# Enigmatisms/Distributed-Machine-Learning-Experiment-Document

Measured on AMD Instinct MI355X. Metric: samples/sec (whole node) for task3 DDP CNN at 1/2/4/8 MI355X, higher is better.
Workload: dtype bf16; 1 GPU; model=resnet18, global_batch=1024, per_gpu_batch=1024, image_size=224, parallelism=dp1, optimizer=SGD(momentum=0.9), fused flat, ddp=none (dp1: no communication), backend=native, fused_step=False, hip_graph=False, stream_priority=high, sampler=MySampler(partition)

## Files before the change

### csrc/stem_fused.hip

```cpp
#include <type_traits>

#include "common.h"
#include "igemm_common.h"
#include "kernels.h"

namespace dm {

namespace {

constexpr int SCO = 64;
constexpr int SKP = 176;
constexpr int SKH = 192;
constexpr int RING = 13;

typedef short s4v __attribute__((ext_vector_type(4)));
typedef unsigned int nt4 __attribute__((ext_vector_type(4)));
typedef unsigned int nt2 __attribute__((ext_vector_type(2)));
__device__ __forceinline__ s4v tr4(const unsigned char* p) {
  return __builtin_amdgcn_ds_read_tr16_b64_v4i16((__attribute__((address_space(3))) s4v*)p);
}

struct StemGeo {
  int Hin, Win, Hout, Wout, PH, PW;
  int ROWB;
  int SP;
};

struct RawUnit {
  uint4 w;
};

__device__ __forceinline__ void lds_barrier() {
  asm volatile("s_waitcnt lgkmcnt(0)\n\ts_barrier" ::: "memory");
}

__device__ __forceinline__ int ring_of(int iy) { return (iy + 13 * 8) % RING; }

template <int NT, int RU>
struct RawMap {
  int r[RU], k[RU];
  unsigned valid;
  float sc[RU][4], bi[RU][4];
  __device__ __forceinline__ void init(int t, int Win, const float (&nsc)[3], const float (&nbi)[3]) {
    const int upr = 3 * Win / 4;
#pragma unroll
    for (int u = 0; u < RU; ++u) {
      const int e = t + NT * u;
      r[u] = e < 4 * upr ? e / upr : -1;
      k[u] = e - (e / upr) * upr;
#pragma unroll
      for (int j = 0; j < 4; ++j) {
        const int c = (k[u] + j) % 3;
        sc[u][j] = c == 0 ? nsc[0] : c == 1 ? nsc[1] : nsc[2];
        bi[u][j] = c == 0 ? nbi[0] : c == 1 ? nbi[1] : nbi[2];
      }
    }
  }
  template <int DT>
  __device__ __forceinline__ void load(RawUnit (&ru)[RU], const void* img, long long rowbase, int Hin,
                                       int Win, int iy0, int nrows) {
    valid = 0;
#pragma unroll
    for (int u = 0; u < RU; ++u) {
      const int iy = iy0 + r[u];
      const bool ok = r[u] >= 0 && r[u] < nrows && iy >= 0 && iy < Hin;
      valid |= ok ? 1u << u : 0u;
      const int iyc = min(max(iy, 0), Hin - 1);
      const long long off = rowbase + (long long)iyc * Win * 3 + 4LL * (r[u] >= 0 ? k[u] : 0);
      if (DT == 0) {
        ru[u].w = *reinterpret_cast<const uint4*>(reinterpret_cast<const float*>(img) + off);
      } else if (DT == 1) {
        const uint2 w = *reinterpret_cast<const uint2*>(reinterpret_cast<const bf16_t*>(img) + off);
        ru[u].w = make_uint4(w.x, w.y, 0, 0);
      } else {
        ru[u].w = make_uint4(*reinterpret_cast<const uint32_t*>(reinterpret_cast<const uint8_t*>(img) + off), 0, 0, 0);
      }
    }
  }
  template <int DT>
  __device__ __forceinline__ void store(const RawUnit (&ru)[RU], bf16_t* S, int SP, int nrows) const {
#pragma unroll
    for (int u = 0; u < RU; ++u) {
      if (r[u] < 0 || r[u] >= nrows) continue;
      float x[4];
      const uint4 w = ru[u].w;
      if (DT == 0) {
        x[0] = __uint_as_float(w.x); x[1] = __uint_as_float(w.y);
        x[2] = __uint_as_float(w.z); x[3] = __uint_as_float(w.w);
      } else if (DT == 1) {
        x[0] = __uint_as_float(w.x << 16); x[1] = __uint_as_float(w.x & 0xffff0000u);
        x[2] = __uint_as_float(w.y << 16); x[3] = __uint_as_float(w.y & 0xffff0000u);
      } else {
        x[0] = (float)(w.x & 0xff); x[1] = (float)((w.x >> 8) & 0xff);
        x[2] = (float)((w.x >> 16) & 0xff); x[3] = (float)(w.x >> 24);
      }
      const bool ok = (valid >> u) & 1;
#pragma unroll
      for (int j = 0; j < 4; ++j) x[j] = ok ? fmaf(x[j], sc[u][j], bi[u][j]) : 0.f;
      bf16_t* p = S + r[u] * SP + 4 * k[u] + 9;
      p[0] = f2bf(x[0]);
      *reinterpret_cast<uint32_t*>(p + 1) = pack_bf2(x[1], x[2]);
      p[3] = f2bf(x[3]);
    }
  }
};

struct EMap {
  bool act;
  int soff, eoff;
  int part;
  __device__ __forceinline__ void init(int t, int Wout) {
    act = t < 3 * Wout;
    const int ox = t / 3;
    part = t - 3 * ox;
    soff = 6 * ox + 8 * part;
    eoff = 48 * ox + 16 * part;
  }
  __device__ __forceinline__ void build(unsigned char* E, const bf16_t* S, const StemGeo& G, int iy0,
                                        int nrows, int srow0) const {
    if (!act) return;
    if (nrows == 4) build_n<4>(E, S, G, iy0, srow0);
    else if (nrows == 2) build_n<2>(E, S, G, iy0, srow0);
    else for (int q = 0; q < nrows; ++q) build_n<1>(E, S, G, iy0 + q, srow0 + q);
  }
  template <int NR>
  __device__ __forceinline__ void build_n(unsigned char* E, const bf16_t* S, const StemGeo& G,
                                          int iy0, int srow0) const {
    uint32_t w[NR][4];
#pragma unroll
    for (int q = 0; q < NR; ++q) {
      const int sr = min(max(srow0 + q, 0), 3);
      const uint32_t* sp = reinterpret_cast<const uint32_t*>(S + sr * G.SP + soff);
#pragma unroll
      for (int j = 0; j < 4; ++j) w[q][j] = sp[j];
    }
#pragma unroll
    for (int q = 0; q < NR; ++q) {
      const int iy = iy0 + q;
      const bool in = iy >= 0 && iy < G.Hin;
      uint4 v = make_uint4(in ? w[q][0] : 0u, in ? w[q][1] : 0u, in ? w[q][2] : 0u, in ? w[q][3] : 0u);
      if (part == 2) {
        v.z = in ? (v.z & 0xffffu) | 0x3f800000u : 0u;
        v.w = 0;
      }
      *reinterpret_cast<uint4*>(E + ring_of(iy) * G.ROWB + eoff) = v;
    }
  }
};

__host__ __device__ constexpr unsigned wcode(int kh, int kw) { return (unsigned)((2 - kh) << 2 | (2 - kw)); }

__device__ __forceinline__ uint32_t mono2(uint32_t w) {
  const uint32_t s = (w >> 15) & 0x00010001u;
  return w ^ (s * 0x7fffu);
}

__device__ __forceinline__ int yoff(int slot, int px, int c8, int Wout) {
  return ((slot * Wout + px) * 8 + (c8 ^ ((((px >> 1) & 1) << 2) | ((px >> 2) & 3)))) * 16;
}

template <int PF>
__device__ __forceinline__ f32x16 conv_tile(const bf16x8 (&wa)[11], const unsigned char* E,
                                            const int (&rowoff)[7], int pxoff, bool hh) {
  f32x16 acc;
#pragma unroll
  for (int r = 0; r < 16; ++r) acc[r] = 0.f;
  bf16x8 bq[11];
#pragma unroll
  for (int s = 0; s < 11 + PF; ++s) {
    if (s < 11) {
      const int j0 = 2 * s, j1 = 2 * s + 1;
      const int k0 = j0 / 3 > 6 ? 6 : j0 / 3, k1 = j1 / 3 > 6 ? 6 : j1 / 3;
      const int a0 = rowoff[k0] + 16 * (j0 % 3), a1 = rowoff[k1] + 16 * (j1 % 3);
      bq[s] = *reinterpret_cast<const bf16x8*>(E + (hh ? a1 : a0) + pxoff);
    }
    if (s >= PF) acc = __builtin_amdgcn_mfma_f32_32x32x16_bf16(wa[s - PF], bq[s - PF], acc, 0, 0, 0);
  }
  return acc;
}

__device__ __forceinline__ void ring_rows(int (&ro)[7], int iy0, int ROWB) {
  const int r0 = ring_of(iy0);
#pragma unroll
  for (int r = 0; r < 7; ++r) {
    const int x = r0 + r;
    ro[r] = (x >= RING ? x - RING : x) * ROWB;
  }
}

__device__ __forceinline__ void pair_wgrad(f32x16 (&acc)[3], const unsigned char* T,
                                           const unsigned char* E, const StemGeo& G, int i,
                                           int wid, int lane) {
  const int cb = wid & 1, kq = (wid >> 1) & 1;
  const int g = lane >> 4, h = g >> 1, i16 = lane & 15, q = i16 >> 2, p = i16 & 3;
  const int c8 = 4 * cb + 2 * (g & 1) + (p >> 1);
  int ta[2], ta8[2], boff[2][3];
#pragma unroll
  for (int sl = 0; sl < 2; ++sl) {
    ta[sl] = yoff(sl, 4 * h + q, c8, G.Wout) + 8 * (p & 1);
    ta8[sl] = yoff(sl, 4 * h + q + 8, c8, G.Wout) + 8 * (p & 1);
    const int oy = 2 * i + sl;
#pragma unroll
    for (int u = 0; u < 3; ++u) {
      const int k = 32 * (3 * kq + u) + 16 * (g & 1) + 4 * p;
      int ky = k / 24, kk = k - 24 * ky;
      if (ky > 6) ky = 6;
      boff[sl][u] = ring_of(2 * oy - 3 + ky) * G.ROWB + (4 * h + q) * 48 + 2 * kk;
    }
  }
  struct Stage {
    s4v a0, a1, b0[3], b1[3];
  };
  auto load = [&](Stage& S, int t, int sl) {
    const int mo = 16 * t;
    S.a0 = tr4(T + ta[sl] + mo * 128);
    S.a1 = tr4(T + ta8[sl] + mo * 128);
#pragma unroll
    for (int u = 0; u < 3; ++u) {
      S.b0[u] = tr4(E + boff[sl][u] + mo * 48);
      S.b1[u] = tr4(E + boff[sl][u] + (mo + 8) * 48);
    }
  };
  auto mma = [&](const Stage& S) {
    const bf16x8 af = (bf16x8){S.a0[0], S.a0[1], S.a0[2], S.a0[3], S.a1[0], S.a1[1], S.a1[2], S.a1[3]};
#pragma unroll
    for (int u = 0; u < 3; ++u) {
      const bf16x8 bf = (bf16x8){S.b0[u][0], S.b0[u][1], S.b0[u][2], S.b0[u][3],
                                 S.b1[u][0], S.b1[u][1], S.b1[u][2], S.b1[u][3]};
      acc[u] = __builtin_amdgcn_mfma_f32_32x32x16_bf16(af, bf, acc[u], 0, 0, 0);
    }
  };
  const int nt = G.Wout >> 4;
  Stage s0, s1;
  load(s0, 0, 0);
  for (int t = 0; t < nt; ++t) {
    load(s1, t, 1);
    mma(s0);
    if (t + 1 < nt) load(s0, t + 1, 0);
    mma(s1);
  }
}

}

struct StemFwdArgs {
  const void* img;
  const long long* idx;
  float nsc[3], nbi[3];
  const bf16_t* wk;
  const float* gamma;
  bf16_t* pext;
  uint8_t* code;
  float* stats;
  int N, nimg;
  StemGeo G;
};

constexpr int FNT = 768;
constexpr int FVT = FNT - 256;
constexpr int FRU = 2;

template <int DT>
__global__ void __launch_bounds__(FNT, 1) stem_fwd_kernel(StemFwdArgs a) {
  extern __shared__ __attribute__((aligned(16))) unsigned char smem[];
  const StemGeo G = a.G;
  const int YB = 2 * G.Wout * 128;
  const int SB = 4 * G.SP;
  unsigned char* E = smem;
  unsigned char* Y = E + RING * G.ROWB;
  bf16_t* S = reinterpret_cast<bf16_t*>(Y + 2 * YB);
  const int tid = threadIdx.x, lane = tid & 63, wid = tid >> 6;
  const bool train = a.stats != nullptr;
  {
    const int tot16 = (RING * G.ROWB + 2 * YB + 2 * SB * 2) / 16;
    for (int e = tid; e < tot16; e += FNT) reinterpret_cast<uint4*>(smem)[e] = make_uint4(0, 0, 0, 0);
  }
  __syncthreads();
  const int nimg = a.N > (int)blockIdx.x ? (a.N - 1 - (int)blockIdx.x) / (int)gridDim.x + 1 : 0;
  const int SPI = G.PH + 2;
  const int nsteps = nimg * SPI;
  auto img_base = [&](int q) -> long long {
    const int n = (int)blockIdx.x + q * (int)gridDim.x;
    long long row = a.idx ? a.idx[n] : (long long)n;
    row = row < 0 ? 0 : row >= a.nimg ? a.nimg - 1 : row;
    return row * G.Hin * G.Win * 3;
  };
  const bool mw = wid < 4;
  if (mw) {
    const int slot = wid >> 1, cb = wid & 1, hh = lane >> 5;
    bf16x8 wa[11];
#pragma unroll
    for (int s = 0; s < 11; ++s)
      wa[s] = *reinterpret_cast<const bf16x8*>(a.wk + (32 * cb + (lane & 31)) * SKP + 16 * s + 8 * hh);
    uint32_t flm[4][2];
#pragma unroll
    for (int g4 = 0; g4 < 4; ++g4)
#pragma unroll
      for (int h = 0; h < 2; ++h) {
        const int co = 32 * cb + 8 * g4 + 4 * hh + 2 * h;
        flm[g4][h] = (a.gamma[co] < 0.f ? 0xffffu : 0u) | (a.gamma[co + 1] < 0.f ? 0xffff0000u : 0u);
      }
    float st_s[16], st_q[16];
#pragma unroll
    for (int r = 0; r < 16; ++r) st_s[r] = st_q[r] = 0.f;
    for (int st = 0; st <= nsteps; ++st) {
      lds_barrier();
      if (st == nsteps) break;
      const int kk = st % SPI;
      if (kk < 2) continue;
      const int i = kk - 2;
      unsigned char* Yt = Y + (st & 1) * YB;
      int ro[7];
      ring_rows(ro, 4 * i - 3 + 2 * slot, G.ROWB);
#pragma unroll
      for (int mb = 0; mb < 4; ++mb) {
        if (32 * mb >= G.Wout) break;
        const int px = 32 * mb + (lane & 31);
        const int pxb = min(px, G.Wout - 1);
        f32x16 acc = conv_tile<4>(wa, E, ro, pxb * 48, hh);
        const bool valid = px < G.Wout;
        if (32 * mb + 32 > G.Wout) {
#pragma unroll
          for (int r = 0; r < 16; ++r) acc[r] = valid ? acc[r] : 0.f;
        }
#pragma unroll
        for (int r = 0; r < 16; ++r) {
          st_s[r] += acc[r];
          st_q[r] = fmaf(acc[r], acc[r], st_q[r]);
        }
        if (valid) {
#pragma unroll
          for (int g4 = 0; g4 < 4; ++g4) {
            const uint32_t k0 = mono2(pack_bf2(acc[4 * g4 + 0], acc[4 * g4 + 1])) ^ flm[g4][0];
            const uint32_t k1 = mono2(pack_bf2(acc[4 * g4 + 2], acc[4 * g4 + 3])) ^ flm[g4][1];
            *reinterpret_cast<uint2*>(Yt + yoff(slot, px, 4 * cb + g4, G.Wout) + 8 * hh) = make_uint2(k0, k1);
          }
        }
      }
    }
    if (!train) return;
    float* red = reinterpret_cast<float*>(smem);
    __syncthreads();
#pragma unroll
    for (int r = 0; r < 16; ++r) {
      red[((wid * 2 + 0) * 16 + r) * 64 + lane] = st_s[r];
      red[((wid * 2 + 1) * 16 + r) * 64 + lane] = st_q[r];
    }
    __syncthreads();
    if (tid < 2 * SCO) {
      const int co = tid & 63, which = tid >> 6;
      const int c = co >> 5, cl = co & 31, h = (cl >> 2) & 1, r = (cl & 3) + 4 * (cl >> 3);
      float sum = 0.f;
      for (int sl = 0; sl < 2; ++sl) {
        const float* rp = red + (((2 * sl + c) * 2 + which) * 16 + r) * 64 + 32 * h;
        for (int l = 0; l < 32; ++l) sum += rp[l];
      }
      a.stats[(long long)blockIdx.x * 2 * SCO + which * SCO + co] = sum;
    }
    return;
  }
  const int vt = tid - 256;
  RawMap<FVT, FRU> rm;
  rm.init(vt, G.Win, a.nsc, a.nbi);
  EMap em;
  em.init(vt, G.Wout);
  RawUnit ru[FRU];
  const bool pact = vt < G.PW * 8;
  const int pj = vt >> 3, pc8 = vt & 7;
  uint32_t pflip[4];
#pragma unroll
  for (int k = 0; k < 4; ++k) {
    const int c = pc8 * 8 + 2 * k;
    pflip[k] = (pact && a.gamma[c] < 0.f ? 0xffffu : 0u) |
               (pact && a.gamma[c + 1] < 0.f ? 0xffff0000u : 0u);
  }
  int pv[8];
  long long bcur = nimg > 0 ? img_base(0) : 0, bnext = nimg > 1 ? img_base(1) : 0;
  int bq = 0;
  auto base = [&](int qq) {
    if (qq != bq) {
      bcur = bnext;
      bq = qq;
      bnext = qq + 1 < nimg ? img_base(qq + 1) : 0;
    }
    return bcur;
  };
  auto plan = [&](int t, int& pq, int& piy) -> int {
    if (t >= nsteps) return 0;
    pq = t / SPI;
    const int k = t - pq * SPI;
    if (k == 0) { piy = 0; return 4; }
    if (k == 1) { piy = 4; return 2; }
    if (k - 2 + 1 < G.PH) { piy = 4 * (k - 2) + 6; return 4; }
    return 0;
  };
  int pend = 0;
  if (nimg > 0) {
    rm.load<DT>(ru, a.img, bcur, G.Hin, G.Win, 0, 4);
    rm.store<DT>(ru, S + 1 * SB, G.SP, 4);
    int pq = 0, piy = 0;
    pend = plan(1, pq, piy);
    if (pend) rm.load<DT>(ru, a.img, base(pq), G.Hin, G.Win, piy, pend);
  }
  for (int st = 0; st <= nsteps; ++st) {
    lds_barrier();
    const int q = st / SPI, kk = st - q * SPI;
    if (pend) rm.store<DT>(ru, S + (st & 1) * SB, G.SP, pend);
    {
      int pq = 0, piy = 0;
      pend = plan(st + 2, pq, piy);
      if (pend) rm.load<DT>(ru, a.img, base(pq), G.Hin, G.Win, piy, pend);
    }
    if (st >= 1) {
      const int ps = st - 1, pq = ps / SPI, pk = ps - pq * SPI;
      if (pk >= 2 && pact) {
        const int i = pk - 2;
        const unsigned char* Yt = Y + (ps & 1) * YB;
        if (i == 0) {
#pragma unroll
          for (int c = 0; c < 8; ++c) pv[c] = INT_MIN;
        }
        int hk[2][8];
#pragma unroll
        for (int sl = 0; sl < 2; ++sl) {
          uint4 w[3];
#pragma unroll
          for (int kw = 0; kw < 3; ++kw) {
            const int px = 2 * pj - 1 + kw;
            w[kw] = (px >= 0 && px < G.Wout) ? *reinterpret_cast<const uint4*>(Yt + yoff(sl, px, pc8, G.Wout))
                                             : make_uint4(0x80008000u, 0x80008000u, 0x80008000u, 0x80008000u);
          }
#pragma unroll
          for (int c = 0; c < 8; ++c) {
            const int sh = 16 * (c & 1);
            int k3[3];
#pragma unroll
            for (int kw = 0; kw < 3; ++kw) {
              const uint32_t ww[4] = {w[kw].x, w[kw].y, w[kw].z, w[kw].w};
              const uint32_t d = ww[c >> 1];
              k3[kw] = (int)((sh ? (d & 0xffff0000u) : (d << 16)) | (uint32_t)(2 - kw));
            }
            hk[sl][c] = max(max(k3[0], k3[1]), k3[2]);
          }
        }
        uint32_t o[4] = {0, 0, 0, 0}, cd = 0;
#pragma unroll
        for (int c = 0; c < 8; ++c) {
          const int v = max(max(pv[c] | 8, hk[0][c] | 4), hk[1][c]);
          cd |= ((uint32_t)v & 15u) << (4 * c);
          o[c >> 1] |= ((uint32_t)v >> 16) << (16 * (c & 1));
          pv[c] = hk[1][c];
        }
#pragma unroll
        for (int k = 0; k < 4; ++k) o[k] = mono2(o[k] ^ pflip[k]);
        const int n = (int)blockIdx.x + pq * (int)gridDim.x;
        const long long po = (((long long)n * G.PH + i) * G.PW + pj) * SCO + pc8 * 8;
        __builtin_nontemporal_store((nt4){o[0], o[1], o[2], o[3]}, reinterpret_cast<nt4*>(a.pext + po));
        __builtin_nontemporal_store(cd, reinterpret_cast<uint32_t*>(a.code + po / 2));
      }
    }
    if (st < nsteps) {
      const bf16_t* Sp = S + ((st - 1) & 1) * SB;
      if (kk == 0) em.build(E, Sp, G, -3, 7, -3);
      else if (kk == 1) em.build(E, Sp, G, 4, 2, 0);
      else if (kk - 2 + 1 < G.PH) em.build(E, Sp, G, 4 * (kk - 2) + 6, 4, 0);
    }
  }
  if (train) {
    __syncthreads();
    __syncthreads();
  }
}

__global__ void __launch_bounds__(256) stem_pool_apply_kernel(const bf16_t* __restrict__ pext,
                                                              const uint32_t* __restrict__ code,
                                                              const float* __restrict__ scale,
                                                              const float* __restrict__ shift,
                                                              bf16_t* __restrict__ out,
                                                              uint32_t* __restrict__ code4,
                                                              long long n8) {
  constexpr int U = 4;
  const long long b = (long long)blockIdx.x * 256 * U + threadIdx.x;
  nt4 v[U];
  uint32_t cd[U];
#pragma unroll
  for (int u = 0; u < U; ++u) {
    const long long e = b + 256LL * u;
    if (e < n8) {
      v[u] = __builtin_nontemporal_load(reinterpret_cast<const nt4*>(pext) + e);
      cd[u] = code4 ? __builtin_nontemporal_load(code + e) : 0u;
    }
  }
#pragma unroll
  for (int u = 0; u < U; ++u) {
    const long long e = b + 256LL * u;
    if (e >= n8) continue;
    const int c0 = (int)(e & 7) * 8;
    const uint32_t w[4] = {v[u][0], v[u][1], v[u][2], v[u][3]};
    uint32_t o[4], keep = 0;
#pragma unroll
    for (int k = 0; k < 4; ++k) {
      float r[2];
#pragma unroll
      for (int hlf = 0; hlf < 2; ++hlf) {
        const int c = c0 + 2 * k + hlf;
        const float z = bf2f((bf16_t)((w[k] >> (16 * hlf)) & 0xffff)) * scale[c] + shift[c];
        r[hlf] = z > 0.f ? z : 0.f;
        keep |= z > 0.f ? 15u << (4 * (2 * k + hlf)) : 0u;
      }
      o[k] = pack_bf2(r[0], r[1]);
    }
    __builtin_nontemporal_store((nt4){o[0], o[1], o[2], o[3]}, reinterpret_cast<nt4*>(out) + e);
    if (code4) code4[e] = (cd[u] & keep) | ~keep;
  }
}

constexpr int GK = 192;
constexpr int GONE = 93;
struct WavePlan {
  int nb, blk[4];
  int tcb;
  int nt, kind[5], x[5], y[5];
};
__device__ constexpr WavePlan kPlans[8] = {
    {2, {0, 1, 0, 0}, 0, 5, {0, 0, 0, 1, 1}, {0, 0, 1, 0, 0}, {0, 1, 1, 0, 1}},
    {2, {2, 3, 0, 0}, 0, 5, {0, 0, 0, 1, 1}, {0, 0, 1, 0, 0}, {0, 1, 1, 0, 1}},
    {2, {4, 5, 0, 0}, 0, 5, {0, 0, 0, 1, 1}, {0, 0, 1, 0, 0}, {0, 1, 1, 0, 1}},
    {4, {0, 1, 2, 3}, -1, 4, {0, 0, 0, 0, 0}, {0, 0, 1, 1, 0}, {2, 3, 2, 3, 0}},
    {4, {0, 1, 4, 5}, -1, 4, {0, 0, 0, 0, 0}, {0, 0, 1, 1, 0}, {2, 3, 2, 3, 0}},
    {4, {2, 3, 4, 5}, -1, 4, {0, 0, 0, 0, 0}, {0, 0, 1, 1, 0}, {2, 3, 2, 3, 0}},
    {3, {0, 1, 2, 0}, 1, 3, {1, 1, 1, 0, 0}, {0, 0, 0, 0, 0}, {0, 1, 2, 0, 0}},
    {3, {3, 4, 5, 0}, 1, 3, {1, 1, 1, 0, 0}, {0, 0, 0, 0, 0}, {0, 1, 2, 0, 0}},
};

struct BwdFrags {
  bf16x8 xf[4], tf;
};

template <int W>
__device__ __forceinline__ void gram_slot(f32x16 (&acc)[5], const unsigned char* T,
                                          const unsigned char* E, const StemGeo& G, int i,
                                          int slot, int t0, int t1, int lane) {
  constexpr WavePlan P = kPlans[W];
  const int g = lane >> 4, h = g >> 1, i16 = lane & 15, q = i16 >> 2, p = i16 & 3;
  const int oy = 2 * i + slot;
  int boff[4];
#pragma unroll
  for (int b = 0; b < P.nb; ++b) {
    const int k = 32 * P.blk[b] + 16 * (g & 1) + 4 * p;
    int ky = k / 24;
    const int kk = k - 24 * ky;
    if (ky > 6) ky = 6;
    boff[b] = ring_of(2 * oy - 3 + ky) * G.ROWB + (4 * h + q) * 48 + 2 * kk;
  }
  int ta = 0, ta8 = 0;
  if (P.tcb >= 0) {
    const int c8 = 4 * P.tcb + 2 * (g & 1) + (p >> 1);
    ta = yoff(slot, 4 * h + q, c8, G.Wout) + 8 * (p & 1);
    ta8 = yoff(slot, 4 * h + q + 8, c8, G.Wout) + 8 * (p & 1);
  }
  auto load = [&](BwdFrags& F, int t) {
    const int mo = 16 * t;
#pragma unroll
    for (int b = 0; b < P.nb; ++b) {
      const s4v v0 = tr4(E + boff[b] + mo * 48), v1 = tr4(E + boff[b] + (mo + 8) * 48);
      F.xf[b] = (bf16x8){v0[0], v0[1], v0[2], v0[3], v1[0], v1[1], v1[2], v1[3]};
    }
    if (P.tcb >= 0) {
      const s4v v0 = tr4(T + ta + mo * 128), v1 = tr4(T + ta8 + mo * 128);
      F.tf = (bf16x8){v0[0], v0[1], v0[2], v0[3], v1[0], v1[1], v1[2], v1[3]};
    }
  };
  auto mma = [&](const BwdFrags& F) {
#pragma unroll
    for (int j = 0; j < P.nt; ++j)
      acc[j] = __builtin_amdgcn_mfma_f32_32x32x16_bf16(P.kind[j] ? F.tf : F.xf[P.x[j]], F.xf[P.y[j]],
                                                       acc[j], 0, 0, 0);
  };
  for (int t = t0; t < t1; ++t) {
    BwdFrags f;
    load(f, t);
    mma(f);
  }
}

template <int W>
__device__ __forceinline__ void gram_store(const f32x16 (&acc)[5], float* dslab, float* gslab,
                                           int lane) {
  constexpr WavePlan P = kPlans[W];
#pragma unroll
  for (int j = 0; j < P.nt; ++j)
#pragma unroll
    for (int r = 0; r < 16; ++r) {
      const int row = (r & 3) + 8 * (r >> 2) + 4 * (lane >> 5);
      const int col = 32 * P.blk[P.y[j]] + (lane & 31);
      if (P.kind[j])
        dslab[(long long)blockIdx.x * SCO * SKH + (32 * P.tcb + row) * SKH + col] = acc[j][r];
      else
        gslab[(long long)blockIdx.x * GK * GK + (32 * P.blk[P.x[j]] + row) * GK + col] = acc[j][r];
    }
}

template <int W>
__device__ __forceinline__ void gram_zero(f32x16 (&acc)[5]) {
#pragma unroll
  for (int j = 0; j < 5; ++j)
#pragma unroll
    for (int r = 0; r < 16; ++r) acc[j][r] = 0.f;
}

struct StemBwdArgs2 {
  const void* img;
  const long long* idx;
  float nsc[3], nbi[3];
  const bf16_t* wk;
  const bf16_t* pdy;
  const uint8_t* code4;
  float* dslab;
  float* gslab;
  int N, nimg;
  int split;
  StemGeo G;
};

constexpr int PRING = 3;
constexpr int BNT = 1024;
constexpr int BMW = 8;
constexpr int BVT = BNT - 64 * BMW;

template <int DT>
__global__ void __launch_bounds__(BNT, 1) stem_bwd_kernel(StemBwdArgs2 a) {
  extern __shared__ __attribute__((aligned(16))) unsigned char smem[];
  const StemGeo G = a.G;
  const int TB = 2 * G.Wout * 128;
  unsigned char* E = smem;
  unsigned char* T = E + RING * G.ROWB;
  bf16_t* S = reinterpret_cast<bf16_t*>(T + 2 * TB);
  const int PRB = G.PW * SCO;
  bf16_t* Pg = S + 4 * G.SP;
  uint8_t* Pc = reinterpret_cast<uint8_t*>(Pg + PRING * PRB);
  const int tid = threadIdx.x, lane = tid & 63, wid = tid >> 6;
  {
    const int tot16 = (RING * G.ROWB + 2 * TB + 4 * G.SP * 2) / 16;
    for (int e = tid; e < tot16; e += BNT) reinterpret_cast<uint4*>(smem)[e] = make_uint4(0, 0, 0, 0);
  }
  const int nimg = a.N > (int)blockIdx.x ? (a.N - 1 - (int)blockIdx.x) / (int)gridDim.x + 1 : 0;
  const int SPI = G.PH + 2;
  const int nsteps = nimg * SPI;
  auto img_of = [&](int q) { return (int)blockIdx.x + q * (int)gridDim.x; };
  auto img_base = [&](int q) -> long long {
    long long row = a.idx ? a.idx[img_of(q)] : (long long)img_of(q);
    row = row < 0 ? 0 : row >= a.nimg ? a.nimg - 1 : row;
    return row * G.Hin * G.Win * 3;
  };
  if (wid < BMW) {
    f32x16 acc[5];
    gram_zero<0>(acc);
    __syncthreads();
    EMap em;
    em.init(tid, G.Wout);
    auto run = [&](auto wtag) {
      constexpr int W = decltype(wtag)::value;
      for (int st = 0; st <= nsteps; ++st) {
        lds_barrier();
        const int ps = st - 1;
        const int pk = ps >= 0 ? ps % SPI : -1;
        const bool work = ps >= 0 && pk >= 2;
        const unsigned char* Tt = T + (ps & 1) * TB;
        const int nt = G.Wout >> 4, split = min(a.split, 2 * nt);
        if (work) {
          gram_slot<W>(acc, Tt, E, G, pk - 2, 0, 0, min(split, nt), lane);
          if (split > nt) gram_slot<W>(acc, Tt, E, G, pk - 2, 1, 0, split - nt, lane);
        }
        lds_barrier();
        if (work) {
          if (split < nt) gram_slot<W>(acc, Tt, E, G, pk - 2, 0, split, nt, lane);
          gram_slot<W>(acc, Tt, E, G, pk - 2, 1, max(split - nt, 0), nt, lane);
        }
        if (st < nsteps) {
          const int kk = st % SPI;
          if (kk == 1) em.build(E, S, G, -3, 5, -3);
          else if (kk >= 2) em.build(E, S, G, 4 * (kk - 2) + 2, 4, 0);
        }
      }
      gram_store<W>(acc, a.dslab, a.gslab, lane);
    };
    switch (wid) {
      case 0: run(std::integral_constant<int, 0>{}); break;
      case 1: run(std::integral_constant<int, 1>{}); break;
      case 2: run(std::integral_constant<int, 2>{}); break;
      case 3: run(std::integral_constant<int, 3>{}); break;
      case 4: run(std::integral_constant<int, 4>{}); break;
      case 5: run(std::integral_constant<int, 5>{}); break;
      case 6: run(std::integral_constant<int, 6>{}); break;
      default: run(std::integral_constant<int, 7>{}); break;
    }
    return;
  }
  const int vt = tid - 64 * BMW;
  RawMap<BVT, FRU> rm;
  rm.init(vt, G.Win, a.nsc, a.nbi);
  RawUnit ru[FRU];
  const bool pl = vt < G.PW * 8;
  uint4 pg_r;
  uint32_t pc_r;
  bool p_ok = false;
  auto pload = [&](int q, int r) {
    p_ok = pl && r < G.PH;
    const int rc = min(r, G.PH - 1), vc = pl ? vt : 0;
    const long long o = (((long long)img_of(min(q, nimg - 1)) * G.PH + rc) * G.PW) * SCO + vc * 8;
    pg_r = *reinterpret_cast<const uint4*>(a.pdy + o);
    pc_r = *reinterpret_cast<const uint32_t*>(a.code4 + o / 2);
  };
  auto pstore = [&](int r) {
    if (!pl) return;
    const int sl = r % PRING;
    *reinterpret_cast<uint4*>(Pg + sl * PRB + vt * 8) = p_ok ? pg_r : make_uint4(0, 0, 0, 0);
    *reinterpret_cast<uint32_t*>(Pc + (sl * PRB + vt * 8) / 2) = p_ok ? pc_r : 0xffffffffu;
  };
  const int qb = vt >> 3, qc = vt & 7, c0 = qc * 8;
  __syncthreads();
  const bool colok = qb + 1 < G.PW;
  const int ocol0 = qb * SCO + c0, ocol1 = (colok ? qb + 1 : qb) * SCO + c0;
  int toff[4];
#pragma unroll
  for (int pp = 0; pp < 4; ++pp) toff[pp] = yoff(pp >> 1, 2 * qb + (pp & 1), qc, G.Wout);
  uint2 gres[4];
  auto gquad = [&](uint2 (&res)[4], int i, int hf) {
    uint2 qg[4];
    uint32_t qi[4];
    const int sl0 = i % PRING, sl1 = sl0 + 1 == PRING ? 0 : sl0 + 1;
    const bool rowok = i + 1 < G.PH;
#pragma unroll
    for (int w = 0; w < 4; ++w) {
      const int wa = w >> 1, wb = w & 1;
      const int o = (wa ? sl1 : sl0) * PRB + (wb ? ocol1 : ocol0);
      qg[w] = *reinterpret_cast<const uint2*>(Pg + o + 4 * hf);
      const uint32_t c = *reinterpret_cast<const uint16_t*>(Pc + o / 2 + 2 * hf);
      qi[w] = ((wa && !rowok) || (wb && !colok)) ? 0xffffu : c;
    }
#pragma unroll
    for (int pp = 0; pp < 4; ++pp) {
      const int ddy = pp >> 1, ddx = pp & 1;
      float d[4] = {0.f, 0.f, 0.f, 0.f};
#pragma unroll
      for (int w = 0; w < 4; ++w) {
        const int wa = w >> 1, wb = w & 1;
        if ((wa && !ddy) || (wb && !ddx)) continue;
        const uint32_t gw[2] = {qg[w].x, qg[w].y};
        const unsigned code = wcode(ddy ? (wa ? 0 : 2) : 1, ddx ? (wb ? 0 : 2) : 1);
#pragma unroll
        for (int j = 0; j < 4; ++j) {
          const uint32_t g = gw[j >> 1];
          const float gf = __uint_as_float((j & 1) ? (g & 0xffff0000u) : (g << 16));
          d[j] += (qi[w] & (15u << (4 * j))) == (code << (4 * j)) ? gf : 0.f;
        }
      }
      res[pp] = make_uint2(pack_bf2(d[0], d[1]), pack_bf2(d[2], d[3]));
    }
  };


  long long bcur = nimg > 0 ? img_base(0) : 0, bnext = nimg > 1 ? img_base(1) : 0;
  int bq = 0;
  auto base = [&](int qq) {
    if (qq != bq) {
      bcur = bnext;
      bq = qq;
      bnext = qq + 1 < nimg ? img_base(qq + 1) : 0;
    }
    return bcur;
  };
  for (int st = 0; st <= nsteps; ++st) {
    const int q = st / SPI, kk = st - q * SPI;
    lds_barrier();
    if (st < nsteps) {
      if (kk == 0) {
        pload(q, 0);
        pstore(0);
        pload(q, 1);
        pstore(1);
        pload(q, 2);
      } else if (kk == 1) {
        rm.store<DT>(ru, S, G.SP, 2);
      } else {
        const int i = kk - 2;
        pstore(i + 2);
        pload(q, i + 3);
        rm.store<DT>(ru, S, G.SP, 4);
        if (pl) gquad(gres, i, 0);
      }
    }
    lds_barrier();
    if (st < nsteps) {
      if (kk == 0) {
        rm.load<DT>(ru, a.img, base(q), G.Hin, G.Win, 0, 2);
      } else if (kk == 1) {
        rm.load<DT>(ru, a.img, base(q), G.Hin, G.Win, 2, 4);
      } else {
        const int i = kk - 2;
        if (pl) {
          uint2 r1[4];
          gquad(r1, i, 1);
          unsigned char* Tt = T + (st & 1) * TB;
#pragma unroll
          for (int pp = 0; pp < 4; ++pp)
            *reinterpret_cast<uint4*>(Tt + toff[pp]) = make_uint4(gres[pp].x, gres[pp].y, r1[pp].x, r1[pp].y);
        }
        if (i + 1 < G.PH) rm.load<DT>(ru, a.img, base(q), G.Hin, G.Win, 4 * i + 6, 4);
      }
    }
  }
}

__global__ void __launch_bounds__(256) stem_slab_reduce_kernel(const float* __restrict__ dslab,
                                                               const float* __restrict__ gslab,
                                                               int GD, float* __restrict__ dsum,
                                                               float* __restrict__ gsum) {
  const int e = blockIdx.x * 256 + threadIdx.x;
  const int nd = SCO * SKH, ng = GK * GK;
  if (e >= nd + ng) return;
  const float* src = e < nd ? dslab + e : gslab + (e - nd);
  const long long stride = e < nd ? nd : ng;
  float s4[4] = {0.f, 0.f, 0.f, 0.f};
  int gi = 0;
  for (; gi + 4 <= GD; gi += 4)
#pragma unroll
    for (int u = 0; u < 4; ++u) s4[u] += src[(long long)(gi + u) * stride];
  for (; gi < GD; ++gi) s4[0] += src[(long long)gi * stride];
  const float v = (s4[0] + s4[1]) + (s4[2] + s4[3]);
  if (e < nd) dsum[e] = v;
  else gsum[e - nd] = v;
}

__global__ void __launch_bounds__(256) stem_wcombine_kernel(const float* __restrict__ dsum,
                                                            const float* __restrict__ gsum,
                                                            const bf16_t* __restrict__ wk,
                                                            const float* __restrict__ coef,
                                                            float* __restrict__ dw, float beta) {
  __shared__ float wrow[SKP];
  const int co = blockIdx.x, t = threadIdx.x;
  for (int k = t; k < SKP; k += 256) wrow[k] = bf2f(wk[co * SKP + k]);
  __syncthreads();
  if (t >= 147) return;
  const int ky = t / 21, rem = t - 21 * ky, kx = rem / 3, c = rem - 3 * kx;
  const int k = ky * 24 + kx * 3 + c;
  float wg = 0.f;
  for (int j = 0; j < SKP; ++j) {
    const float gv = j <= k ? gsum[j * GK + k] : gsum[k * GK + j];
    wg = fmaf(wrow[j], gv, wg);
  }
  const float colsum = GONE <= k ? gsum[GONE * GK + k] : gsum[k * GK + GONE];
  const float d = coef[co] * dsum[co * SKH + k] + coef[SCO + co] * wg + coef[2 * SCO + co] * colsum;
  float* o = dw + ((co * 3 + c) * 7 + ky) * 7 + kx;
  *o = (beta != 0.f ? beta * *o : 0.f) + d;
}

__global__ void __launch_bounds__(256) stem_pack_weights_kernel(const float* __restrict__ w,
                                                                bf16_t* __restrict__ wk) {
  const int e = blockIdx.x * 256 + threadIdx.x;
  if (e >= SCO * SKP) return;
  const int co = e / SKP, k = e - co * SKP;
  const int ky = k / 24, kk = k - 24 * ky, kx = kk / 3, c = kk - 3 * kx;
  float v = 0.f;
  if (ky < 7 && kk < 21) v = w[((co * 3 + c) * 7 + ky) * 7 + kx];
  wk[e] = f2bf(v);
}

static StemGeo stem_geo(int Hin, int Win) {
  StemGeo G;
  G.Hin = Hin;
  G.Win = Win;
  G.Hout = Hin / 2;
  G.Wout = Win / 2;
  G.PH = G.Hout / 2;
  G.PW = G.Wout / 2;
  G.ROWB = G.Wout * 48;
  G.SP = 3 * Win + 24;
  return G;
}

bool stem_fused_supported(int Hin, int Win) {
  return Hin >= 8 && Hin % 4 == 0 && Win % 32 == 0 && Win <= 224;
}

static size_t fwd_smem(const StemGeo& G) {
  const size_t tiles = (size_t)RING * G.ROWB + (size_t)2 * 2 * G.Wout * 128 + (size_t)2 * 4 * G.SP * 2;
  const size_t red = (size_t)4 * 2 * 16 * 64 * 4;
  return tiles > red ? tiles : red;
}
static size_t bwd_smem(const StemGeo& G) {
  return (size_t)RING * G.ROWB + (size_t)2 * 2 * G.Wout * 128 + (size_t)4 * G.SP * 2 +
         (size_t)PRING * G.PW * SCO * 2 + (size_t)PRING * G.PW * SCO / 2;
}

int stem_fused_grid(int N) {
  static int cus = 0;
  if (!cus) {
    int dev = 0;
    DM_CHECK(hipGetDevice(&dev));
    DM_CHECK(hipDeviceGetAttribute(&cus, hipDeviceAttributeMultiprocessorCount, dev));
  }
  return N < cus ? N : cus;
}

void stem_fwd_fused(const void* img, int dtype, const long long* idx, const float* nsc,
                    const float* nbi, const bf16_t* wk, const float* gamma, bf16_t* pext,
                    uint8_t* code, float* stats, int N, int nimg, int Hin, int Win, int grid,
                    hipStream_t st) {
  StemFwdArgs a;
  a.img = img;
  a.idx = idx;
  for (int c = 0; c < 3; ++c) {
    a.nsc[c] = nsc[c];
    a.nbi[c] = nbi[c];
  }
  a.wk = wk;
  a.gamma = gamma;
  a.pext = pext;
  a.code = code;
  a.stats = stats;
  a.N = N;
  a.nimg = nimg;
  a.G = stem_geo(Hin, Win);
  const size_t sm = fwd_smem(a.G);
#define DM_SF(DT)                                              \
  do {                                                         \
    set_smem_attr(stem_fwd_kernel<DT>, sm);                    \
    stem_fwd_kernel<DT><<<grid, FNT, sm, st>>>(a);             \
  } while (0)
  if (dtype == 0) DM_SF(0);
  else if (dtype == 1) DM_SF(1);
  else DM_SF(2);
#undef DM_SF
  DM_CHECK(hipGetLastError());
}

void stem_pool_apply(const bf16_t* pext, const uint8_t* code, const float* scale,
                     const float* shift, bf16_t* out, uint8_t* code4, long long n, hipStream_t st) {
  const long long n8 = n / 8;
  stem_pool_apply_kernel<<<(unsigned)((n8 + 1023) / 1024), 256, 0, st>>>(
      pext, reinterpret_cast<const uint32_t*>(code), scale, shift, out,
      reinterpret_cast<uint32_t*>(code4), n8);
  DM_CHECK(hipGetLastError());
}

void stem_bwd_fused2(const void* img, int dtype, const long long* idx, const float* nsc,
                     const float* nbi, const bf16_t* wk, const bf16_t* pdy, const uint8_t* code4,
                     float* dslab, float* gslab, int N, int nimg, int Hin, int Win, int grid,
                     hipStream_t st) {
  StemBwdArgs2 a;
  a.img = img;
  a.idx = idx;
  for (int c = 0; c < 3; ++c) {
    a.nsc[c] = nsc[c];
    a.nbi[c] = nbi[c];
  }
  a.wk = wk;
  a.pdy = pdy;
  a.code4 = code4;
  a.dslab = dslab;
  a.gslab = gslab;
  a.N = N;
  a.nimg = nimg;
  a.G = stem_geo(Hin, Win);
  a.split = (2 * (a.G.Wout >> 4) * 5 + 6) / 7;
  const size_t sm = bwd_smem(a.G);
#define DM_SB(DT)                                              \
  do {                                                         \
    set_smem_attr(stem_bwd_kernel<DT>, sm);                    \
    stem_bwd_kernel<DT><<<grid, BNT, sm, st>>>(a);             \
  } while (0)
  if (dtype == 0) DM_SB(0);
  else if (dtype == 1) DM_SB(1);
  else DM_SB(2);
#undef DM_SB
  DM_CHECK(hipGetLastError());
}

void stem_wcombine(const float* dslab, const float* gslab, int GD, const bf16_t* wk,
                   const float* coef, float* sums, float* dw, float beta, hipStream_t st) {
  const int n = SCO * SKH + GK * GK;
  float* dsum = sums;
  float* gsum = sums + SCO * SKH;
  stem_slab_reduce_kernel<<<(n + 255) / 256, 256, 0, st>>>(dslab, gslab, GD, dsum, gsum);
  DM_CHECK(hipGetLastError());
  stem_wcombine_kernel<<<SCO, 256, 0, st>>>(dsum, gsum, wk, coef, dw, beta);
  DM_CHECK(hipGetLastError());
}
int stem_gram_cols() { return GK; }
int stem_sums_len() { return SCO * SKH + GK * GK; }

void stem_pack_weights(const float* w, bf16_t* wk, hipStream_t st) {
  stem_pack_weights_kernel<<<(SCO * SKP + 255) / 256, 256, 0, st>>>(w, wk);
  DM_CHECK(hipGetLastError());
}

int stem_slab_cols() { return SKH; }
int stem_wk_cols() { return SKP; }

}
```

Baseline: 56030 samples/s.

## Software-pipeline stem conv MFMA with epilogue interleaving and packed bf16 stats

Restructures the stem conv producer warps so all column blocks run as one flattened, statically unrolled MFMA stream, specialised on the number of 32-pixel blocks. LDS fragment loads are prefetched three steps ahead, and each block's epilogue (BN stats, bf16 pack, monotone key transform, LDS store) is interleaved slice-by-slice with the next block's MFMAs using double-buffered accumulators and sched barriers. Packing and stats use 2-wide vector ops. The aim is to hide epilogue and load latency behind matrix work, at the cost of higher register pressure and a fragile hand-tuned schedule.

```diff
diff --git a/csrc/stem_fused.hip b/csrc/stem_fused.hip
--- a/csrc/stem_fused.hip
+++ b/csrc/stem_fused.hip
@@ -155,28 +155,31 @@
   return w ^ (s * 0x7fffu);
 }
 
+typedef float f32x2 __attribute__((ext_vector_type(2)));
+typedef __bf16 bf16x2v __attribute__((ext_vector_type(2)));
+typedef short s16x2 __attribute__((ext_vector_type(2)));
+__device__ __forceinline__ uint32_t pack_bf2v(float lo, float hi) {
+  return __builtin_bit_cast(uint32_t, __builtin_convertvector((f32x2){lo, hi}, bf16x2v));
+}
+__device__ __forceinline__ uint32_t mono2v(uint32_t w) {
+  const s16x2 neg = __builtin_bit_cast(s16x2, w) >> 15;
+  return w ^ (__builtin_bit_cast(uint32_t, neg) & 0x7fff7fffu);
+}
+
 __device__ __forceinline__ int yoff(int slot, int px, int c8, int Wout) {
   return ((slot * Wout + px) * 8 + (c8 ^ ((((px >> 1) & 1) << 2) | ((px >> 2) & 3)))) * 16;
 }
 
-template <int PF>
-__device__ __forceinline__ f32x16 conv_tile(const bf16x8 (&wa)[11], const unsigned char* E,
-                                            const int (&rowoff)[7], int pxoff, bool hh) {
-  f32x16 acc;
-#pragma unroll
-  for (int r = 0; r < 16; ++r) acc[r] = 0.f;
-  bf16x8 bq[11];
-#pragma unroll
-  for (int s = 0; s < 11 + PF; ++s) {
-    if (s < 11) {
-      const int j0 = 2 * s, j1 = 2 * s + 1;
-      const int k0 = j0 / 3 > 6 ? 6 : j0 / 3, k1 = j1 / 3 > 6 ? 6 : j1 / 3;
-      const int a0 = rowoff[k0] + 16 * (j0 % 3), a1 = rowoff[k1] + 16 * (j1 % 3);
-      bq[s] = *reinterpret_cast<const bf16x8*>(E + (hh ? a1 : a0) + pxoff);
-    }
-    if (s >= PF) acc = __builtin_amdgcn_mfma_f32_32x32x16_bf16(wa[s - PF], bq[s - PF], acc, 0, 0, 0);
-  }
-  return acc;
+constexpr int FBLK = 32 * 48;
+__device__ __forceinline__ void frag_offsets(int (&fa)[11], const int (&rowoff)[7], int pxoff,
+                                             bool hh) {
+#pragma unroll
+  for (int s = 0; s < 11; ++s) {
+    const int j0 = 2 * s, j1 = 2 * s + 1;
+    const int k0 = j0 / 3 > 6 ? 6 : j0 / 3, k1 = j1 / 3 > 6 ? 6 : j1 / 3;
+    const int a0 = rowoff[k0] + 16 * (j0 % 3), a1 = rowoff[k1] + 16 * (j1 % 3);
+    fa[s] = (hh ? a1 : a0) + pxoff;
+  }
 }
 
 __device__ __forceinline__ void ring_rows(int (&ro)[7], int iy0, int ROWB) {
@@ -300,51 +303,99 @@
         const int co = 32 * cb + 8 * g4 + 4 * hh + 2 * h;
         flm[g4][h] = (a.gamma[co] < 0.f ? 0xffffu : 0u) | (a.gamma[co + 1] < 0.f ? 0xffff0000u : 0u);
       }
-    float st_s[16], st_q[16];
-#pragma unroll
-    for (int r = 0; r < 16; ++r) st_s[r] = st_q[r] = 0.f;
-    for (int st = 0; st <= nsteps; ++st) {
-      lds_barrier();
-      if (st == nsteps) break;
-      const int kk = st % SPI;
-      if (kk < 2) continue;
-      const int i = kk - 2;
-      unsigned char* Yt = Y + (st & 1) * YB;
-      int ro[7];
-      ring_rows(ro, 4 * i - 3 + 2 * slot, G.ROWB);
-#pragma unroll
-      for (int mb = 0; mb < 4; ++mb) {
-        if (32 * mb >= G.Wout) break;
-        const int px = 32 * mb + (lane & 31);
-        const int pxb = min(px, G.Wout - 1);
-        f32x16 acc = conv_tile<4>(wa, E, ro, pxb * 48, hh);
+    f32x2 st_s[8], st_q[8];
+#pragma unroll
+    for (int j = 0; j < 8; ++j) st_s[j] = st_q[j] = (f32x2){0.f, 0.f};
+    constexpr int YBLK = 32 * 128;
+    const int l31 = lane & 31;
+    int yo[4];
+#pragma unroll
+    for (int g4 = 0; g4 < 4; ++g4) yo[g4] = yoff(slot, l31, 4 * cb + g4, G.Wout) + 8 * hh;
+    auto run = [&](auto nbtag) {
+      constexpr int NB = decltype(nbtag)::value, NT = 11 * NB, PF = 3;
+      for (int st = 0; st <= nsteps; ++st) {
+        lds_barrier();
+        if (st == nsteps) break;
+        const int kk = st % SPI;
+        if (kk < 2) continue;
+        const int i = kk - 2;
+        unsigned char* Yt = Y + (st & 1) * YB;
+        int ro[7], fa[11];
+        ring_rows(ro, 4 * i - 3 + 2 * slot, G.ROWB);
+        frag_offsets(fa, ro, l31 * 48, hh);
+#pragma unroll
+        for (int s = 0; s < 11; ++s) asm volatile("" : "+v"(fa[s]));
+        f32x16 acc[2];
+        bf16x8 bq[NT];
+        uint32_t k0 = 0;
+        auto stat = [&](const f32x16& c, int j) {
+          const f32x2 v = (f32x2){c[2 * j], c[2 * j + 1]};
+          st_s[j] += v;
+          st_q[j] = __builtin_elementwise_fma(v, v, st_q[j]);
+        };
+        auto slice = [&](const f32x16& c, int mb, int s) {
+          if (s < 1 || s > 8) return;
+          const int g4 = (s - 1) >> 1, h = (s - 1) & 1;
+          const uint32_t k = mono2v(pack_bf2v(c[4 * g4 + 2 * h], c[4 * g4 + 2 * h + 1])) ^ flm[g4][h];
+          if (h == 0) {
+            k0 = k;
+            asm volatile("" : "+v"(k0));
+          } else {
+            *reinterpret_cast<uint2*>(Yt + yo[g4] + YBLK * mb) = make_uint2(k0, k);
+          }
+          stat(c, s - 1);
+          asm volatile("" : "+v"(st_s[s - 1]), "+v"(st_q[s - 1]));
+        };
+#pragma unroll
+        for (int t = 0; t < (PF < NT ? PF : NT); ++t)
+          bq[t] = *reinterpret_cast<const bf16x8*>(E + fa[t % 11] + FBLK * (t / 11));
+        __builtin_amdgcn_sched_barrier(0);
+#pragma unroll
+        for (int t = 0; t < NT; ++t) {
+          const int mb = t / 11, s = t % 11;
+          f32x16& c = acc[mb & 1];
+          if (s == 0) {
+#pragma unroll
+            for (int r = 0; r < 16; ++r) c[r] = 0.f;
+          }
+          c = __builtin_amdgcn_mfma_f32_32x32x16_bf16(wa[s], bq[t], c, 0, 0, 0);
+          if (t + PF < NT)
+            bq[t + PF] = *reinterpret_cast<const bf16x8*>(E + fa[(t + PF) % 11] + FBLK * ((t + PF) / 11));
+          if (mb >= 1) slice(acc[(mb - 1) & 1], mb - 1, s);
+          __builtin_amdgcn_sched_barrier(0);
+        }
+        f32x16& c = acc[(NB - 1) & 1];
+        const int px = 32 * (NB - 1) + l31;
         const bool valid = px < G.Wout;
-        if (32 * mb + 32 > G.Wout) {
-#pragma unroll
-          for (int r = 0; r < 16; ++r) acc[r] = valid ? acc[r] : 0.f;
+        if (32 * NB > G.Wout) {
+#pragma unroll
+          for (int r = 0; r < 16; ++r) c[r] = valid ? c[r] : 0.f;
         }
 #pragma unroll
-        for (int r = 0; r < 16; ++r) {
-          st_s[r] += acc[r];
-          st_q[r] = fmaf(acc[r], acc[r], st_q[r]);
-        }
+        for (int j = 0; j < 8; ++j) stat(c, j);
         if (valid) {
 #pragma unroll
           for (int g4 = 0; g4 < 4; ++g4) {
-            const uint32_t k0 = mono2(pack_bf2(acc[4 * g4 + 0], acc[4 * g4 + 1])) ^ flm[g4][0];
-            const uint32_t k1 = mono2(pack_bf2(acc[4 * g4 + 2], acc[4 * g4 + 3])) ^ flm[g4][1];
-            *reinterpret_cast<uint2*>(Yt + yoff(slot, px, 4 * cb + g4, G.Wout) + 8 * hh) = make_uint2(k0, k1);
+            const uint32_t ka = mono2v(pack_bf2v(c[4 * g4 + 0], c[4 * g4 + 1])) ^ flm[g4][0];
+            const uint32_t kb = mono2v(pack_bf2v(c[4 * g4 + 2], c[4 * g4 + 3])) ^ flm[g4][1];
+            *reinterpret_cast<uint2*>(Yt + yo[g4] + YBLK * (NB - 1)) = make_uint2(ka, kb);
           }
         }
       }
+    };
+    switch ((G.Wout + 31) >> 5) {
+      case 1: run(std::integral_constant<int, 1>{}); break;
+      case 2: run(std::integral_constant<int, 2>{}); break;
+      case 3: run(std::integral_constant<int, 3>{}); break;
+      default: run(std::integral_constant<int, 4>{}); break;
     }
     if (!train) return;
     float* red = reinterpret_cast<float*>(smem);
     __syncthreads();
 #pragma unroll
     for (int r = 0; r < 16; ++r) {
-      red[((wid * 2 + 0) * 16 + r) * 64 + lane] = st_s[r];
-      red[((wid * 2 + 1) * 16 + r) * 64 + lane] = st_q[r];
+      red[((wid * 2 + 0) * 16 + r) * 64 + lane] = st_s[r >> 1][r & 1];
+      red[((wid * 2 + 1) * 16 + r) * 64 + lane] = st_q[r >> 1][r & 1];
     }
     __syncthreads();
     if (tid < 2 * SCO) {
```

Measured after the change: 56190 samples/s (median of 5 runs). About the same (+0.3%).
